# nquach/TEE_optical_flow

Hardware: AMD Instinct MI355X
Metric: frame-pairs/sec @512x512 DualTVL1 (higher is better)
Workload: dtype f32

## Files before the change

### tee_optical_flow_amd/csrc/teeflow.hip

```cpp
#include "teeflow_kernels.hip.h"
#include "teeflow_deepflow.hip.h"
#include "teeflow_sor_rt.hip.h"
#include "teeflow_analysis.hip.h"
#include "teeflow_wase.hip.h"
#include "teeflow_saliency.hip.h"
#include "teeflow_ccl.hip.h"
#include "teeflow_masks.hip.h"
#include "teeflow_otsu.hip.h"
#include "teeflow_centroid.hip.h"
#include "teeflow_area.hip.h"
#include "teeflow_polar.hip.h"
#include "teeflow_overlay.hip.h"
#include "teeflow_magoverlay.hip.h"
#include "teeflow_segmentor.hip.h"
#include "teeflow_inflate.hip.h"
#include "teeflow_deflate.hip.h"
#include "teeflow_ingest.hip.h"
#include "pil_resample_tables.h"
#include "../../include/teeflow.h"
#include "teeflow_engine.hip.h"
#include "teeflow_tvl1_host.hip.h"
#include "teeflow_deepflow_host.hip.h"
#include "teeflow_queue.hip.h"

// ... 102 lines not shown
        case TF_PARAM_EPSILON: *d = &p.epsilon; break;
        case TF_PARAM_INNER_ITERATIONS: *i = &p.inner_iterations; break;
        case TF_PARAM_OUTER_ITERATIONS: *i = &p.outer_iterations; break;
        case TF_PARAM_SCALE_STEP: *d = &p.scale_step; break;
        case TF_PARAM_GAMMA: *d = &p.gamma; break;
        case TF_PARAM_MEDIAN_FILTERING: *i = &p.median_filtering; break;
        case TF_PARAM_USE_INITIAL_FLOW: *i = &p.use_initial_flow; break;
        default: return false;
    }
    return true;
}

TF_API int tf_set_param(tf_handle* h, int key, double v)
{
    if (!h) return TF_ERR_INVALID_ARG;
    if (h->P.algo == TF_ALGO_DEEPFLOW) return fail(h, TF_ERR_UNSUPPORTED, "DeepFlow handles have creation-time parameters only (as cv2's object)");
    tf_params p = h->P;
    double* d; int* i;
    if (!param_field(p, key, &d, &i)) return fail(h, TF_ERR_INVALID_ARG, "unknown parameter key %d", key);
    if (d) *d = v; else *i = key == TF_PARAM_USE_INITIAL_FLOW ? v != 0.0 : (int)v;
    int rc = validate_params(h, p);
    if (rc) return rc;
    h->P = p;
    return TF_OK;
}

TF_API int tf_get_param(tf_handle* h, int key, double* v)
{
    if (!h || !v) return TF_ERR_INVALID_ARG;
    double* d; int* i;
    if (!param_field(h->P, key, &d, &i)) return fail(h, TF_ERR_INVALID_ARG, "unknown parameter key %d", key);
    *v = d ? *d : *i;
    return TF_OK;
}

TF_API int tf_set_stream(tf_handle* h, void* hip_stream, int use_external)
{
    if (!h) return TF_ERR_INVALID_ARG;
    HIPC(h, hipStreamSynchronize(h->stream));
    h->stream = use_external ? (hipStream_t)hip_stream : h->own_stream;
    return TF_OK;
}

TF_API int tf_set_tuning(tf_handle* h, const char* name, int value)
{
    if (!h || !name) return TF_ERR_INVALID_ARG;
    const std::string n(name);
    if (n == "iter_variant") {
        if (value < 0 || value > 2) return fail(h, TF_ERR_UNSUPPORTED, "iter_variant must be 0 (64x16 tiles), 1 (row strips) or 2 (row strips, two iterations per launch), got %d", value);
        h->iter_variant = value;
    }
    else if (n == "strip_blocks") h->strip_blocks = value > 0 ? value : 2048;
    else if (n == "min_rows_work") h->min_rows_work = value;
    else if (n == "lane_slots_pct") h->lane_slots_pct = value;
    else if (n == "sor_rt") h->sor_rt = value ? 1 : 0;
    else if (n == "sor_rt_shape") h->sor_rt_shape = value;
    else if (n == "sor_plain_div") h->sor_plain_div = value ? 1 : 0;
    else if (n == "max_strip_width") h->max_strip_width = value < 4 ? 4 : (value > 2048 ? 2048 : value);
    else if (n == "lanes") h->lanes = value < 1 ? 1 : (value > 8 ? 8 : value);
    else if (n == "queue_lanes") h->queue_lanes = value;
    else if (n == "queue_unit") h->queue_unit = value < 0 ? 0 : value;
    else if (n == "queue_test_fail_unit") h->queue_test_fail_unit = value;
    else if (n == "sor_fuse") h->sor_fuse = value;
    else if (n == "sor_coop") {
        h->sor_coop = value;
        if (value) { h->coop.rearm(); ++h->sor_coop_arm; }
    }
    else if (n == "sor_coop_s") h->sor_coop_s = value;
    else if (n == "sor_coop_small") h->sor_coop_small = value ? 1 : 0;
    else if (n == "sor_coop_min_util") h->sor_coop_min_util = value;
    else if (n == "coop_test_mute") h->coop_test_mute = value ? 1 : 0;
    else if (n == "coop_test_occ16") { h->coop_test_occ16 = value; h->coop.occ16 = -1; if (h->coop.flags) h->coop.query_occupancy(*h); }
    else if (n == "coop_test_occ8") { h->coop_test_occ8 = value; h->coop.occ16 = -1; if (h->coop.flags) h->coop.query_occupancy(*h); }
    else if (n == "coop_backoff") { h->coop.backoff = value < 0 ? 0 : value; }
    else if (n == "df_fuse_ds") h->df_fuse_ds = value < 0 ? 0 : (value > 2 ? 2 : value);
    else if (n == "warp_margin") h->warp_margin = value < 0 ? 0 : (value > 40 ? 40 : value);
    else if (n == "overlay_chunk_kib") h->overlay_chunk_kib = value < 0 ? 0 : (value > (512 << 10) ? (512 << 10) : value);
    else if (n == "area_chunk_kib") h->area_chunk_kib = value < 0 ? 0 : (value > (512 << 10) ? (512 << 10) : value);
    else return fail(h, TF_ERR_INVALID_ARG, "unknown tuning knob %s", name);
    return TF_OK;
}

#ifdef TF_COOP_TIMING
extern "C" __attribute__((visibility("default"))) int tf_dbg_coop_times(unsigned long long* out)
{
    return (int)hipMemcpyFromSymbol(out, HIP_SYMBOL(g_coop_t), sizeof(unsigned long long) * 4 * 64);
}
#endif
TF_API long long tf_dbg_counter(tf_handle* h, const char* name)
{
    if (!h || !name) return -1;
    const std::string n(name);
    long long v = -1;
    std::vector<CoopCounters> all{h->coop.counters()};
    if (h->pool) { std::lock_guard<std::mutex> lk(h->pool->m); all.insert(all.end(), h->pool->coop.begin(), h->pool->coop.end()); }
    if (n == "coop_launches") { v = 0; for (auto& c : all) v += c.launches; }
    else if (n == "coop_aborts") { v = 0; for (auto& c : all) v += c.aborts; }
    else if (n == "coop_disabled") { v = 0; for (auto& c : all) v |= (long long)c.disabled; }
    else if (n == "coop_rearms") { v = 0; for (auto& c : all) v += c.rearms; }
    else if (n == "coop_cooldown") { v = 0; for (auto& c : all) v = v > c.cooldown ? v : c.cooldown; }
    else if (n == "saliency_kernel_us") v = (long long)(h->pre_kernel_ms * 1000.0);
    else if (n == "wase_study_kernel_us") v = (long long)(h->wase_kernel_ms * 1000.0);
    else if (n == "inflate_kernel_us") v = (long long)(h->inflate_kernel_ms * 1000.0);
    else if (n == "unchunk_kernel_us") v = (long long)(h->unchunk_kernel_ms * 1000.0);
    else if (n == "deflate_match_us") v = (long long)(h->deflate_match_ms * 1000.0);
    else if (n == "deflate_emit_us") v = (long long)(h->deflate_emit_ms * 1000.0);
// ... 258 lines not shown
```

### tee_optical_flow_amd/csrc/teeflow_dbg.hip.h

```cpp
namespace {
template <class T> struct DevBuf { T* p = nullptr; ~DevBuf() { if (p) (void)hipFree(p); } };
using DBuf = DevBuf<float>;

int dbg_up(tf_handle* h, DBuf& d, const float* src, const Geom& g)
{
    HIPC(h, hipMalloc(&d.p, (size_t)g.plane * sizeof(float)));
    HIPC(h, hipMemsetAsync(d.p, 0, (size_t)g.plane * sizeof(float), h->stream));
    if (src) HIPC(h, hipMemcpy2DAsync(d.p, (size_t)g.pitch * 4, src, (size_t)g.w * 4, (size_t)g.w * 4, g.h, hipMemcpyHostToDevice, h->stream));
    return TF_OK;
}
int dbg_down(tf_handle* h, float* dst, const float* d, const Geom& g)
{
    HIPC(h, hipMemcpy2DAsync(dst, (size_t)g.w * 4, d, (size_t)g.pitch * 4, (size_t)g.w * 4, g.h, hipMemcpyDeviceToHost, h->stream));
    HIPC(h, hipStreamSynchronize(h->stream));
    return TF_OK;
}

int dbg_up2(tf_handle* h, DBuf& fr, const float* I0, const float* I1, const Geom& g)
{
    HIPC(h, hipMalloc(&fr.p, 2 * (size_t)g.plane * sizeof(float)));
    HIPC(h, hipMemsetAsync(fr.p, 0, 2 * (size_t)g.plane * sizeof(float), h->stream));
    HIPC(h, hipMemcpy2DAsync(fr.p, (size_t)g.pitch * 4, I0, (size_t)g.w * 4, (size_t)g.w * 4, g.h, hipMemcpyHostToDevice, h->stream));
    HIPC(h, hipMemcpy2DAsync(fr.p + g.plane, (size_t)g.pitch * 4, I1, (size_t)g.w * 4, (size_t)g.w * 4, g.h, hipMemcpyHostToDevice, h->stream));
    return TF_OK;
// ... 230 lines not shown
    const Geom g = make_geom(w, hgt);
    DBuf a0, a1, b0, b1;
    int rc;
    if ((rc = dbg_up(h, a0, src, g)) || (rc = dbg_up(h, a1, nullptr, g)) || (rc = dbg_up(h, b0, src, g)) || (rc = dbg_up(h, b1, nullptr, g))) return rc;
    DevBuf<PairCtl> ctl;
    HIPC(h, hipMalloc(&ctl.p, sizeof(PairCtl)));
    HIPC(h, hipMemsetAsync(ctl.p, 0, sizeof(PairCtl), h->stream));
    MedArgs ma = {};
    ma.sb.u1[0] = a0.p; ma.sb.u1[1] = a1.p; ma.sb.u2[0] = b0.p; ma.sb.u2[1] = b1.p;
    ma.ctl = ctl.p; ma.err = nullptr; ma.errstride = 0; ma.it = 0; ma.thr_q = 0; ma.utog = 0; ma.g = g;
    ma.total = 1; ma.step = iter_step(h, false, h->P.inner_iterations);
    const dim3 gm((g.w + 63) / 64, (g.h + 15) / 16, 2);
    if (ksize == 5) hipLaunchKernelGGL(k_median<5>, gm, dim3(256), 0, h->stream, ma);
    else hipLaunchKernelGGL(k_median<3>, gm, dim3(256), 0, h->stream, ma);
    hipError_t e = hipStreamSynchronize(h->stream);
    if (e != hipSuccess) return fail(h, TF_ERR_HIP, "k_median: %s", hipGetErrorString(e));
    return dbg_down(h, dst, a1.p, g);
}

TF_API int tf_dbg_iterate(tf_handle* h, const float* I1wx, const float* I1wy, const float* rho_c,
                          float* u1, float* u2, float* p11, float* p12, float* p21, float* p22,
                          int w, int hgt, int nsteps, int p_is_zero, unsigned long long* err_q)
{
    if (!h || !I1wx || !I1wy || !rho_c || !u1 || !u2 || !p11 || !p12 || !p21 || !p22 || w < 1 || hgt < 1 || nsteps < 0)
        return TF_ERR_INVALID_ARG;
    HIPC(h, hipSetDevice(h->dev));
    const Geom g = make_geom(w, hgt);
    DBuf cx, cy, cr, s[12];
    int rc;
    if ((rc = dbg_up(h, cx, I1wx, g)) || (rc = dbg_up(h, cy, I1wy, g)) || (rc = dbg_up(h, cr, rho_c, g))) return rc;
    float* hostp[6] = {u1, u2, p11, p12, p21, p22};
    for (int k = 0; k < 6; ++k) {
        if ((rc = dbg_up(h, s[2 * k], hostp[k], g)) || (rc = dbg_up(h, s[2 * k + 1], nullptr, g))) return rc;
    }
    DevBuf<PairCtl> ctl; DevBuf<u64> errs;
    HIPC(h, hipMalloc(&ctl.p, sizeof(PairCtl)));
    HIPC(h, hipMemsetAsync(ctl.p, 0, sizeof(PairCtl), h->stream));
    HIPC(h, hipMalloc(&errs.p, (size_t)(nsteps + 1) * sizeof(u64)));
    HIPC(h, hipMemsetAsync(errs.p, 0, (size_t)(nsteps + 1) * sizeof(u64), h->stream));
    Iter2Args A = {};
    IterArgs& ia = A.a;
    ia.wx = cx.p; ia.wy = cy.p; ia.rho = cr.p;
    for (int k = 0; k < 2; ++k) {
        ia.sb.u1[k] = s[0 + k].p; ia.sb.u2[k] = s[2 + k].p; ia.sb.p11[k] = s[4 + k].p;
        ia.sb.p12[k] = s[6 + k].p; ia.sb.p21[k] = s[8 + k].p; ia.sb.p22[k] = s[10 + k].p;
    }
    ia.ctl = ctl.p; ia.err = errs.p; ia.errstride = nsteps + 1; ia.thr_q = -1.0; ia.g = g; ia.host_slot = nullptr; ia.B = 1;
    ia.l_t = (float)(h->P.lambda * h->P.theta); ia.theta = (float)h->P.theta; ia.taut = (float)(h->P.tau / h->P.theta);
    const int step = iter_step(h, false, nsteps);
    A.total = nsteps;
    int launches = 0;
    for (int it = 0; it < nsteps; it += step, ++launches) {
        ia.it = it; ia.utog = ia.ptog = launches; ia.pzero = (p_is_zero && it == 0) ? 1 : 0;
        launch_iter(h, A, step, 1, h->stream);
    }
    hipError_t e = hipStreamSynchronize(h->stream);
    if (e == hipSuccess && err_q && nsteps > 0) {
        e = hipMemcpyAsync(err_q, errs.p, (size_t)nsteps * sizeof(u64), hipMemcpyDeviceToHost, h->stream);
        if (e == hipSuccess) e = hipStreamSynchronize(h->stream);
    }
    if (e != hipSuccess) return fail(h, TF_ERR_HIP, "k_iter: %s", hipGetErrorString(e));
    const int cur = launches & 1;
    for (int k = 0; k < 6; ++k)
        if ((rc = dbg_down(h, hostp[k], s[2 * k + cur].p, g))) return rc;
    return TF_OK;
}
```

### tee_optical_flow_amd/csrc/teeflow_engine.hip.h

```cpp
#include <rccl/rccl.h>
#include <algorithm>
#include <chrono>
#include <cmath>
#include <limits>
#include <cstdarg>
#include <cstdio>
#include <cstring>
#include <cstdlib>
#include <deque>
#include <string>
#include <atomic>
#include <condition_variable>
#include <mutex>
#include <thread>
#include <map>
#include <vector>

#define TF_API extern "C" __attribute__((visibility("default")))

namespace {
constexpr int MAXLEV = 64;
constexpr int DF_MAXLEV = 201;
constexpr int SLOT_RING = 1024;
constexpr int DEFAULT_LAG = 1;
constexpr int DEFAULT_MAX_BATCH = 128;

thread_local std::string g_create_error;

struct ProfEv { hipEvent_t a, b; int level = 0, warp = 0, it = 0; float ms = 0.f; double work = 0.0; };
}

namespace { struct Engine; }
struct LanePool;
struct QJob;
struct CoopCounters { long long launches = 0; int aborts = 0, rearms = 0, cooldown = 0; bool disabled = false; };
struct TfKnobs {
    int iter_variant = 2;
    int max_strip_width = 2048;
    int sor_rt = 1;
    int sor_plain_div = 0;
    int sor_rt_shape = 3;
    int df_fuse_ds = 2;
    int sor_coop = 1;
    int sor_coop_min_util = 85;
    int sor_coop_small = 1;
    int sor_coop_s = 5;
    int sor_fuse = 5;
    int warp_margin = 8;
    int min_rows_work = 8192;
    int strip_blocks = 2048;
    int lane_slots_pct = 67;
    int coop_test_occ16 = -1, coop_test_occ8 = -1;
    int coop_test_mute = 0;
    int profile = 0;
    int overlay_chunk_kib = 0;
    int area_chunk_kib = 0;
    unsigned sor_coop_arm = 0;
};

namespace {
struct Tvl1State {
    int H = 0, W = 0, cap = 0, nlev = 0;
    double scale_step = 0; int nscales = 0, variant = 0;
    Geom lv[MAXLEV];
    float* pyr[MAXLEV] = {};
    float* gxl[MAXLEV] = {}; float* gyl[MAXLEV] = {};
    float *cwx = nullptr, *cwy = nullptr, *crho = nullptr;
    StateBufs sb = {};
    PairCtl* ctl = nullptr;
    u64* errs = nullptr; int errstride = 0;
    int* iters_dev = nullptr; size_t iters_cap = 0;
    const void** chain_src = nullptr; size_t chain_src_cap = 0;
    volatile int* slots_host = nullptr; int* slots_dev = nullptr;
    unsigned launch_seq = 0;
    float* tab = nullptr;
    std::map<size_t, int> slots_cache;
    int ensure(Engine* e, int H, int W, int B);
    void release();
};

struct DfState {
    int nlev = 0, H = 0, W = 0, cap = 0;
    Geom lv[DF_MAXLEV];
    float* pyr_base = nullptr; size_t pyr_off[DF_MAXLEV] = {};
    float* tmp = nullptr;
    float* planes = nullptr;
    DfBufs bufs = {};
    int ensure(Engine* e, int H, int W, int B);
    void release();
};

struct Coop {
    int share = 0;
    bool disabled = false;
    int backoff = 0;
    int cooldown = 0;
    int rearms = 0;
    int occ16 = -1, occ8 = -1;
    int asked16 = -2, asked8 = -2;
    bool used = false;
    int aborts = 0;
    long long launches = 0;
    unsigned epoch = 0;
    unsigned* flags = nullptr;
    int flag_lines = 0;
    void tick();
    void query_occupancy(const TfKnobs& k);
    int ensure(Engine* e);
    int aborted(Engine* e, bool* aborted);
    void rearm() { disabled = false; backoff = cooldown = 0; }
    CoopCounters counters() const { return {launches, aborts, rearms, cooldown, disabled}; }
    void release();
};

struct Engine : TfKnobs {
    tf_params P;
    tf_deepflow_params DP = {};
    int dev = 0;
    int num_cus = 256;
    hipStream_t own_stream = nullptr, stream = nullptr;
    std::string err;
    hipStream_t copy_stream = nullptr;
    hipEvent_t cev[4] = {nullptr, nullptr, nullptr, nullptr};
    uint8_t* st_u8 = nullptr; size_t st_u8_bytes = 0;
    uint8_t* st_flow = nullptr; size_t st_flow_bytes = 0;
    uint8_t* st_init = nullptr; size_t st_init_bytes = 0;
    hipEvent_t ev[4] = {};
// ... 214 lines not shown
```

### tee_optical_flow_amd/csrc/teeflow_tvl1_host.hip.h

```cpp
namespace {
int validate_params(Engine* h, const tf_params& p)
{
    if (p.algo != TF_ALGO_TVL1) return fail(h, TF_ERR_UNSUPPORTED, "algo %d not implemented (only TF_ALGO_TVL1)", p.algo);
    if (p.nscales < 1 || p.nscales > MAXLEV) return fail(h, TF_ERR_INVALID_ARG, "nscales must be in [1,%d], got %d", MAXLEV, p.nscales);
    if (p.warps < 1) return fail(h, TF_ERR_INVALID_ARG, "warps must be >= 1, got %d", p.warps);
    if (p.inner_iterations < 1 || p.outer_iterations < 1)
        return fail(h, TF_ERR_INVALID_ARG, "inner/outer iterations must be >= 1, got %d/%d", p.inner_iterations, p.outer_iterations);
    if ((long long)p.inner_iterations * p.outer_iterations > 100000)
        return fail(h, TF_ERR_INVALID_ARG, "inner*outer iterations too large");
    if (p.median_filtering != 1 && p.median_filtering != 3 && p.median_filtering != 5)
        return fail(h, TF_ERR_UNSUPPORTED, "medianFiltering must be 1, 3 or 5 (cv::medianBlur on CV_32F), got %d", p.median_filtering);
    if (p.gamma != 0.0) return fail(h, TF_ERR_UNSUPPORTED, "gamma != 0 (illumination term u3) is not implemented");
    if (p.variant != TF_VARIANT_CPU && p.variant != TF_VARIANT_CUDA) return fail(h, TF_ERR_INVALID_ARG, "variant must be TF_VARIANT_CPU or TF_VARIANT_CUDA, got %d", p.variant);
    if (p.variant == TF_VARIANT_CUDA && (p.inner_iterations * p.outer_iterations) % 2 != 0)
        return fail(h, TF_ERR_UNSUPPORTED, "TF_VARIANT_CUDA needs an even iteration count (inner*outer), got %d", p.inner_iterations * p.outer_iterations);
    if (p.use_initial_flow && p.variant == TF_VARIANT_CUDA)
        return fail(h, TF_ERR_UNSUPPORTED, "useInitialFlow is not implemented for TF_VARIANT_CUDA (nothing checks that form bit for bit)");
    if (!(p.scale_step > 0.0 && p.scale_step < 1.0)) return fail(h, TF_ERR_INVALID_ARG, "scaleStep must be in (0,1), got %g", p.scale_step);
    if (p.scale_step == 0.5) return fail(h, TF_ERR_UNSUPPORTED, "scaleStep == 0.5 makes cv::resize take its INTER_AREA fast path for the pyramid, which is not implemented");
    if (!(p.theta > 0.0) || !(p.tau > 0.0) || !(p.lambda > 0.0) || !(p.epsilon >= 0.0))
        return fail(h, TF_ERR_INVALID_ARG, "tau, lambda, theta must be > 0 and epsilon >= 0");
    return TF_OK;
}

// ... 32 lines not shown
    HIPC(e, hipStreamSynchronize(e->stream));
    release(); release_staging(e);
    nlev = compute_levels(P, H_, W_, lv);
    const size_t ncap = (size_t)want_cap, fcap = 2 * ncap;
    for (int l = 0; l < nlev; ++l) HIPC(e, hipMalloc(&pyr[l], fcap * lv[l].plane * sizeof(float)));
    if (P.variant == TF_VARIANT_CUDA)
        for (int l = 0; l < nlev; ++l) {
            HIPC(e, hipMalloc(&gxl[l], fcap * lv[l].plane * sizeof(float)));
            HIPC(e, hipMalloc(&gyl[l], fcap * lv[l].plane * sizeof(float)));
        }
    variant = P.variant;
    const size_t pl = (size_t)lv[0].plane * ncap * sizeof(float);
    HIPC(e, hipMalloc(&cwx, pl)); HIPC(e, hipMalloc(&cwy, pl)); HIPC(e, hipMalloc(&crho, pl));
    for (int k = 0; k < 2; ++k) {
        HIPC(e, hipMalloc(&sb.u1[k], pl)); HIPC(e, hipMalloc(&sb.u2[k], pl));
        HIPC(e, hipMalloc(&sb.p11[k], pl)); HIPC(e, hipMalloc(&sb.p12[k], pl));
        HIPC(e, hipMalloc(&sb.p21[k], pl)); HIPC(e, hipMalloc(&sb.p22[k], pl));
    }
    HIPC(e, hipMalloc(&ctl, ncap * sizeof(PairCtl)));
    errstride = total;
    HIPC(e, hipMalloc(&errs, ncap * (size_t)errstride * sizeof(u64)));
    iters_cap = ncap * (size_t)nlev * (size_t)P.warps * 2;
    HIPC(e, hipMalloc(&iters_dev, iters_cap * sizeof(int)));
    H = H_; W = W_; cap = want_cap;
    scale_step = P.scale_step; nscales = P.nscales;
    return TF_OK;
}

inline dim3 grid64x4(const Geom& g, int z) { return dim3((g.w + 63) / 64, (g.h + 3) / 4, z); }

bool rows_ok(const Engine* h, const Geom& g, int B)
{
    return h->iter_variant >= 1 && g.w <= h->max_strip_width && (long long)g.h * B >= h->min_rows_work;
}

int iter_step(const Engine* h, bool cuda_variant, int inner)
{
    return (cuda_variant || (h->iter_variant >= 2 && inner % 2 == 0)) ? 2 : 1;
}

void strip_shape(const Engine* h, const Geom& g, int B, int* R, int* QX, int* RY, int* threads)
{
    const int qx = (g.w + 3) / 4;
    int ry = 256 / qx;
    if (ry < 1) ry = 1;
    *QX = qx; *RY = ry;
    *threads = qx * ry <= 256 ? 256 : (qx * ry + 63) / 64 * 64;
    long long n = (long long)g.h * B / ((long long)h->strip_blocks * ry);
    if (n < 2) n = 2;
    if (n > 16) n = 16;
    *R = ry * (int)n;
}

void launch_iter(Engine* h, const Iter2Args& A, int step, int B, hipStream_t s)
{
    const Geom& g = A.a.g;
    if (!rows_ok(h, g, B)) {
        if (step == 2) hipLaunchKernelGGL(k_iter2_tile, dim3((g.w + T2_OW - 1) / T2_OW, (g.h + T2_OH - 1) / T2_OH, B), dim3(256), 0, s, A);
        else hipLaunchKernelGGL(k_iter, dim3((g.w + IT_OW - 1) / IT_OW, (g.h + IT_OH - 1) / IT_OH, B), dim3(256), 0, s, A.a);
        return;
    }
    int R, QX, RY, threads;
    strip_shape(h, g, B, &R, &QX, &RY, &threads);
    const int LW = QX * 4 + 4;
    if (step == 1) {
        const size_t shmem1 = (size_t)(32 + 8 * RY * LW + 2 * RY * QX) * sizeof(float);
        hipLaunchKernelGGL(k_iter_rows, dim3((g.h + R - 1) / R, 1, B), dim3(threads), shmem1, s, A.a, R, QX, RY);
        return;
    }
    const size_t shmem = (size_t)(32 + 8 * RY * LW + 2 * (RY + 1) * LW + 2 * RY * QX) * sizeof(float);
    if (B <= 1024) {
        auto f = h->tv.slots_cache.find(shmem * 1024 + (size_t)threads / 64);
        if (f == h->tv.slots_cache.end()) {
            int per_cu = 0;
            (void)hipOccupancyMaxActiveBlocksPerMultiprocessor(&per_cu, k_iter2_rows, threads, shmem);
            if (per_cu < 1) per_cu = 1;
            f = h->tv.slots_cache.emplace(shmem * 1024 + (size_t)threads / 64, per_cu * h->num_cus).first;
        }
        int slots = f->second;
        if (h->slots_pct > 0 && h->slots_pct < 100) slots = slots * h->slots_pct / 100;
        int items = 1;
        for (int n = 1; n <= B; ++n) {
            int r, sn;
            strip_rule(n, g.h, RY, slots, &r, &sn);
            if (n * sn > items) items = n * sn;
        }
        hipLaunchKernelGGL(k_iter2_rows, dim3(items, 1, 1), dim3(threads), shmem, s, A, 0, QX, RY, slots);
        return;
    }
    hipLaunchKernelGGL(k_iter2_rows, dim3((g.h + R - 1) / R, 1, B), dim3(threads), shmem, s, A, R, QX, RY, 0);
}

inline int warp_margin_class(int m) { return m <= 0 ? 0 : (m <= 4 ? 4 : (m <= 8 ? 8 : 16)); }
void launch_warp(Engine* h, const WarpArgs& wa, int B, hipStream_t s, const float* gx = nullptr, const float* gy = nullptr)
{
    const Geom& g = wa.g;
    if (h->P.variant == TF_VARIANT_CUDA) {
        WarpCudaArgs ca; ca.w = wa; ca.gx = gx; ca.gy = gy;
        hipLaunchKernelGGL(k_warp_cuda, dim3((g.w + 63) / 64, (g.h + 3) / 4, B), dim3(256), 0, s, ca);
        return;
    }
    const int M = warp_margin_class(h->warp_margin);
    const dim3 grid((g.w + WL_TW - 1) / WL_TW, (g.h + WL_TH - 1) / WL_TH, B);
    const size_t shm = (size_t)(128 + (WL_TW + 2 * (M + 4)) * (WL_TH + 2 * M + 7)) * sizeof(float);
    switch (M) {
        case 4: hipLaunchKernelGGL(k_warp_lds<4>, grid, dim3(256), shm, s, wa); break;
        case 8: hipLaunchKernelGGL(k_warp_lds<8>, grid, dim3(256), shm, s, wa); break;
        case 16: hipLaunchKernelGGL(k_warp_lds<16>, grid, dim3(256), shm, s, wa); break;
        default: hipLaunchKernelGGL(k_warp, dim3((g.w + 63) / 64, (g.h + 3) / 4, B), dim3(256), 0, s, wa); break;
    }
}

int read_reports(Engine* h, hipStream_t s, unsigned q, unsigned* checked, bool* stop)
{
    while (*checked <= q) {
        int v = h->tv.slots_host[*checked % SLOT_RING];
        if (v < 0) {
            if (q - *checked < (unsigned)DEFAULT_LAG) break;
            const double t0 = now_ms();
            while ((v = h->tv.slots_host[*checked % SLOT_RING]) < 0) {
                if (now_ms() - t0 > 20000.0) return fail(h, TF_ERR_HIP, "tvl1_iter launch %u never reported (GPU hang?)", *checked);
                if (hipStreamQuery(s) == hipSuccess && h->tv.slots_host[*checked % SLOT_RING] < 0)
                    return fail(h, TF_ERR_HIP, "stream drained but launch %u did not report", *checked);
            }
        }
        ++*checked;
        if (v == 0) { *stop = true; break; }
    }
    return TF_OK;
}

int run_stage(Engine* h, int l, int wi, int B, int off0, int off1, int* iters_dev)
{
    const tf_params& P = h->P;
    const Geom g = h->tv.lv[l];
    const int inner = P.inner_iterations, total = P.inner_iterations * P.outer_iterations;
    const float thr_f = (float)(P.epsilon * P.epsilon * (double)(g.w * g.h));
    const double thr_q = (double)thr_f * 1073741824.0;
    const double thr_d = P.epsilon * P.epsilon * (double)(g.w * g.h);
    hipStream_t s = h->stream;

    WarpArgs wa;
    wa.pyr = h->tv.pyr[l]; wa.off0 = off0; wa.off1 = off1; wa.sb = h->tv.sb; wa.ctl = h->tv.ctl; wa.tab = h->tv.tab;
    wa.wx = h->tv.cwx; wa.wy = h->tv.cwy; wa.rho = h->tv.crho; wa.g = g;
    int rc = profiled(h, s, -4, 0, 0, [&] { launch_warp(h, wa, B, s, h->tv.gxl[l], h->tv.gyl[l]); });
    if (rc) return rc;
    HIPC(h, hipMemsetAsync(h->tv.errs, 0, (size_t)B * h->tv.errstride * sizeof(u64), s));

    Iter2Args A;
    IterArgs& ia = A.a;
    ia.wx = h->tv.cwx; ia.wy = h->tv.cwy; ia.rho = h->tv.crho; ia.sb = h->tv.sb; ia.ctl = h->tv.ctl; ia.err = h->tv.errs;
    ia.errstride = h->tv.errstride; ia.thr_q = thr_q; ia.g = g;
    ia.l_t = (float)(P.lambda * P.theta); ia.theta = (float)P.theta; ia.taut = (float)(P.tau / P.theta);
    ia.variant = P.variant; ia.thr_d = thr_d;
    const bool cuda_variant = P.variant == TF_VARIANT_CUDA;
    const bool median = P.median_filtering > 1 && !cuda_variant;
    MedArgs ma;
    ma.sb = h->tv.sb; ma.ctl = h->tv.ctl; ma.err = h->tv.errs; ma.errstride = h->tv.errstride; ma.thr_q = thr_q; ma.g = g;

    const dim3 gm((g.w + 63) / 64, (g.h + 15) / 16, 2 * B);
    ia.B = B;
    const int step = iter_step(h, cuda_variant, inner);
    ma.total = A.total = total; ma.step = step;
    A.utog_prev = A.ptog_prev = A.pzero_prev = 0;
    int utog = 0, ptog = 0;
    bool stop = false;
    unsigned checked = h->tv.launch_seq;
    for (int it = 0; it < total + step - 1 && !stop; it += step) {
        if (it < total && it % inner == 0 && median) {
            ma.it = it; ma.utog = utog;
            rc = profiled(h, s, -5, 0, 0, [&] {
                if (P.median_filtering == 5) hipLaunchKernelGGL(k_median<5>, gm, dim3(256), 0, s, ma);
                else hipLaunchKernelGGL(k_median<3>, gm, dim3(256), 0, s, ma);
            });
            if (rc) return rc;
            ++utog;
        }
        const unsigned q = h->tv.launch_seq++;
        h->tv.slots_host[q % SLOT_RING] = -1;
        ia.host_slot = h->tv.slots_dev + q % SLOT_RING;
        ia.it = it; ia.utog = utog; ia.ptog = ptog; ia.pzero = (wi == 0 && it == 0) ? 1 : 0;
        rc = profiled(h, s, l, wi, it, [&] { launch_iter(h, A, step, B, s); });
        if (rc) return rc;
        ++h->tally.iter_launches;
        A.utog_prev = utog; A.ptog_prev = ptog; A.pzero_prev = ia.pzero;
        ++utog; ++ptog;
        rc = read_reports(h, s, q, &checked, &stop);
        if (rc) return rc;
    }
    hipLaunchKernelGGL(k_stage_end, dim3((B + 255) / 256), dim3(256), 0, s, h->tv.errs, h->tv.errstride, h->tv.ctl, iters_dev, B,
                       total, inner, median ? 1 : 0, thr_q, l, wi, h->tv.nlev, P.warps, P.variant, thr_d, step);
    return TF_OK;
}

void pyramids_below_level0(Engine* h, int F)
{
    const tf_params& P = h->P;
    hipStream_t s = h->stream;
    for (int l = 1; l < h->tv.nlev; ++l) {
        const double sc = 1.0 / P.scale_step;
        hipLaunchKernelGGL(k_pyr_down, grid64x4(h->tv.lv[l], F), dim3(256), 0, s, h->tv.pyr[l - 1], h->tv.lv[l - 1], h->tv.pyr[l], h->tv.lv[l], sc, sc,
                           P.variant == TF_VARIANT_CUDA ? 1 : 0);
    }
    if (P.variant == TF_VARIANT_CUDA)
        for (int l = 0; l < h->tv.nlev; ++l)
            hipLaunchKernelGGL(k_grad, grid64x4(h->tv.lv[l], F), dim3(256), 0, s, h->tv.pyr[l], h->tv.gxl[l], h->tv.gyl[l], h->tv.lv[l]);
}

void build_pyramids(Engine* h, const uint8_t* dframes, bool f32, int F)
{
    hipStream_t s = h->stream;
    const Geom g0 = h->tv.lv[0];
    if (f32) hipLaunchKernelGGL(k_f32_to_level0, dim3((g0.w + 255) / 256, g0.h, F), dim3(256), 0, s, (const float*)dframes, h->tv.pyr[0], g0, 1);
    else hipLaunchKernelGGL(k_u8_to_f32, dim3((g0.w + 255) / 256, g0.h, F), dim3(256), 0, s, dframes, h->tv.pyr[0], g0);
    pyramids_below_level0(h, F);
}

enum Seed { SEED_ZERO, SEED_FLOWS, SEED_STATE };

int solve_pairs(Engine* h, int B, int off0, int off1, Seed seed, const float* dinit, int* iters_dev, float scale, void* dflow, bool out_f16)
{
    const tf_params& P = h->P;
    hipStream_t s = h->stream;
    const Geom g0 = h->tv.lv[0];
    const int L = h->tv.nlev - 1;
    const auto seed_step = [&](int l) {
        if (l > 0) hipLaunchKernelGGL(k_init_down, grid64x4(h->tv.lv[l], B), dim3(256), 0, s, h->tv.sb, (L - l + 1) & 1, h->tv.lv[l - 1], h->tv.lv[l],
                                      1.0 / P.scale_step, (float)P.scale_step);
        else if (seed == SEED_FLOWS) hipLaunchKernelGGL(k_init_split, grid64x4(g0, B), dim3(256), 0, s, dinit, h->tv.sb, L & 1, g0);
    };
    if (seed == SEED_STATE)
        hipLaunchKernelGGL(k_chain_seed, dim3((g0.pitch + 63) / 64, (g0.h + 3) / 4, B), dim3(256), 0, s, h->tv.sb, h->tv.ctl, L & 1, g0, L == 0 ? 1 : 0);
    hipLaunchKernelGGL(k_ctl_set, dim3((B + 255) / 256), dim3(256), 0, s, h->tv.ctl, B, 0);
    if (seed != SEED_ZERO) for (int l = 0; l < L; ++l) seed_step(l);
    if (!(seed == SEED_STATE && L == 0)) {
        HIPC(h, hipMemset2DAsync(h->tv.sb.u1[0], (size_t)h->tv.lv[L].splane * sizeof(float), 0, (size_t)h->tv.lv[L].plane * sizeof(float), B, s));
        HIPC(h, hipMemset2DAsync(h->tv.sb.u2[0], (size_t)h->tv.lv[L].splane * sizeof(float), 0, (size_t)h->tv.lv[L].plane * sizeof(float), B, s));
    }
    if (seed != SEED_ZERO) seed_step(L);
    for (int l = L; l >= 0; --l) {
        for (int wi = 0; wi < P.warps; ++wi) {
            int rc = run_stage(h, l, wi, B, off0, off1, iters_dev);
            if (rc) return rc;
        }
        if (l == 0) break;
        const Geom gs = h->tv.lv[l], gd = h->tv.lv[l - 1];
        const double sx = 1.0 / ((double)gd.w / gs.w), sy = 1.0 / ((double)gd.h / gs.h);
        hipLaunchKernelGGL(k_flow_up, grid64x4(gd, B), dim3(256), 0, s, h->tv.sb, h->tv.ctl, gs, gd, sx, sy, (float)(1 / P.scale_step),
                           P.variant == TF_VARIANT_CUDA ? 1 : 0);
        hipLaunchKernelGGL(k_ctl_set, dim3((B + 255) / 256), dim3(256), 0, s, h->tv.ctl, B, 1);
    }
    if (out_f16) hipLaunchKernelGGL(k_output<uint16_t>, out_grid<uint16_t>(g0, B), dim3(256), 0, s, h->tv.sb, h->tv.ctl, g0, scale, (uint16_t*)dflow);
    else hipLaunchKernelGGL(k_output<float>, out_grid<float>(g0, B), dim3(256), 0, s, h->tv.sb, h->tv.ctl, g0, scale, (float*)dflow);
    HIPC(h, hipGetLastError());
    return TF_OK;
}

int solve_resident(Engine* h, const uint8_t* dframes, bool f32, int F, int B, int off0, int off1, float scale, void* dflow, bool out_f16,
                   const float* dinit = nullptr)
{
    build_pyramids(h, dframes, f32, F);
    return solve_pairs(h, B, off0, off1, dinit ? SEED_FLOWS : SEED_ZERO, dinit, h->tv.iters_dev, scale, dflow, out_f16);
}

int solve_chain_resident(Engine* h, const uint8_t* dframes, bool f32, int B, float scale, void* dflow, bool out_f16, bool carry)
{
    build_pyramids(h, dframes, f32, B + 1);
    const size_t per_pair = (size_t)h->tv.nlev * h->P.warps * 2;
    const size_t flb = (size_t)h->tv.H * h->tv.W * 2 * (out_f16 ? sizeof(uint16_t) : sizeof(float));
    for (int k = 0; k < B; ++k) {
        const int rc = solve_pairs(h, 1, k, k + 1, k > 0 || carry ? SEED_STATE : SEED_ZERO, nullptr, h->tv.iters_dev + (size_t)k * per_pair, scale,
                                   (uint8_t*)dflow + (size_t)k * flb, out_f16);
        if (rc) return rc;
        ++h->tally.chain_steps;
    }
    return TF_OK;
}

int solve_chains_resident(Engine* h, const void* const* dsrc, bool f32, int S, int T, const int* Bk, float scale, void* dflow, bool out_f16, bool carry)
{
    const Geom g0 = h->tv.lv[0];
    const int F = (T + 1) * S;
    hipLaunchKernelGGL(k_chain_gather, dim3((g0.w + 255) / 256, g0.h, F), dim3(256), 0, h->stream, dsrc, f32 ? 1 : 0, h->tv.pyr[0], g0);
    pyramids_below_level0(h, F);
    const size_t per_pair = (size_t)h->tv.nlev * h->P.warps * 2;
    const size_t flb = (size_t)h->tv.H * h->tv.W * 2 * (out_f16 ? sizeof(uint16_t) : sizeof(float));
    for (int k = 0; k < T; ++k) {
        const int rc = solve_pairs(h, Bk[k], k * S, (k + 1) * S, k > 0 || carry ? SEED_STATE : SEED_ZERO, nullptr,
                                   h->tv.iters_dev + (size_t)k * S * per_pair, scale, (uint8_t*)dflow + (size_t)k * S * flb, out_f16);
        if (rc) return rc;
        h->tally.chain_steps += Bk[k];
    }
    return TF_OK;
}

void account_bytes(const Engine* h, const int* it , bool seeded, double* iter_bytes, double* total_bytes,
                   unsigned long long* n_in, unsigned long long* n_out)
{
    const int warps = h->P.warps;
    double ib = 0, tb = 0;
    for (int l = 0; l < h->tv.nlev; ++l) {
        const double px = (double)h->tv.lv[l].w * h->tv.lv[l].h;
        for (int w = 0; w < warps; ++w) {
// ... 16 lines not shown
```

### tee_optical_flow_amd/csrc/teeflow_tvl1_iter.hip.h

```cpp
#pragma once

__device__ __forceinline__ bool pair_active(const u64* errb, int it, double thr_q)
{
    if (it == 0) return true;
    return (double)errb[it - 1] > thr_q;
}

#define IT_TW 64
#define IT_TH 16
#define IT_OW 60
#define IT_OH 15

struct IterArgs {
    const float *wx, *wy, *rho;
    StateBufs sb;
    const PairCtl* ctl;
    u64* err; int errstride; int it; double thr_q;
    int utog, ptog, pzero;
    Geom g;
    float l_t, theta, taut;
    int* host_slot;
    int B;
    int variant;
    double thr_d;
// ... 748 lines not shown
                const unsigned mnl = opaque_u(lastrow ? 0u : ~0u);
                float dv1[4], dv2[4], r11[4], r12[4], r21[4], r22[4], u1x[4], u1y[4], u2x[4], u2y[4];
                UNPACK4(dv1, dn1) UNPACK4(dv2, dn2)
                {
                    const float4 o1 = ld4(U2a + (bq * RY + ty) * LW + x), o2 = ld4(U2b + (bq * RY + ty) * LW + x);
                    UNPACK4(s2_u1, o1) UNPACK4(s2_u2, o2)
                }
#pragma unroll
                for (int i = 0; i < 4; ++i) {
                    const float e1 = i < 3 ? s2_u1[i + 1] : rr1, e2 = i < 3 ? s2_u2[i + 1] : rr2;
                    u1x[i] = mask_f(e1 - s2_u1[i], inw[i + 1]);
                    u2x[i] = mask_f(e2 - s2_u2[i], inw[i + 1]);
                    u1y[i] = mask_f(dv1[i] - s2_u1[i], mnl);
                    u2y[i] = mask_f(dv2[i] - s2_u2[i], mnl);
                }
                tv_p_quad_pk(a.taut, u1x, u1y, u2x, u2y, s2_11, s2_12, s2_21, s2_22, r11, r12, r21, r22);
                const size_t prow = (size_t)yc * pitch + x;
                st4(ou1 + prow, PACK4(s2_u1)); st4(ou2 + prow, PACK4(s2_u2));
                st4(o11 + prow, PACK4(r11)); st4(o12 + prow, PACK4(r12));
                st4(o21 + prow, PACK4(r21)); st4(o22 + prow, PACK4(r22));
            }
        }
        else __syncthreads();
        s2_valid = v2u;
#pragma unroll
        for (int i = 0; i < 4; ++i) {
            s2_11[i] = p1_11[i]; s2_12[i] = p1_12[i]; s2_21[i] = p1_21[i]; s2_22[i] = p1_22[i];
            s1_wx[i] = wxv[i]; s1_wy[i] = wyv[i]; s1_r[i] = rv[i];
            s1_11[i] = c11[i]; s1_12[i] = c12[i]; s1_21[i] = c21[i]; s1_22[i] = c22[i];
        }
        s1_valid = v1;
        ring += RY; ring = ring >= RB ? ring - RB : ring;
        if ((s & 255) == 255) { qA += (u64)accA; qB += (u64)accB; accA = accB = 0.0; }
    }
    if (!replay) {
        qA += (u64)accA; qB += (u64)accB;
#pragma unroll
        for (int off = 32; off > 0; off >>= 1) { qA += __shfl_down(qA, off, 64); qB += __shfl_down(qB, off, 64); }
        __syncthreads();
        if ((tid & 63) == 0) { sred[tid >> 6] = qA; sred[8 + (tid >> 6)] = qB; }
        __syncthreads();
        if (tid == 0) {
            u64 ta = 0, tb = 0;
            for (int w = 0; w < (int)(blockDim.x >> 6); ++w) { ta += sred[w]; tb += sred[8 + w]; }
            atomicAdd(&errb[k.it], ta);
            atomicAdd(&errb[k.it + 1], tb);
        }
    }
}

#define T2_OW 52
#define T2_OH 13

__global__ __launch_bounds__(256) void k_iter2_tile(Iter2Args A)
{
    constexpr int LW = 68;
    __shared__ __attribute__((aligned(16))) float sA[16][LW], sB[16][LW];
    __shared__ __attribute__((aligned(16))) float s12[16][LW], s22[16][LW];
    __shared__ float s11w[16][16], s21w[16][16];
    __shared__ u64 sred[8];
    const IterArgs& a = A.a;
    publish_active_count2(A);
    const int b = blockIdx.z;
    u64* errb = a.err + (size_t)b * a.errstride;
    const int mode = pair_mode(errb, a.it, A.total, a.thr_q, a.variant, a.thr_d);
    if (mode == M_EXIT) return;
    const bool replay = mode == M_REPLAY;
    const PairCtl c = a.ctl[b];
    const int utog = replay ? A.utog_prev : a.utog, ptog = replay ? A.ptog_prev : a.ptog;
    const bool pzero = (replay ? A.pzero_prev : a.pzero) != 0;
    const int uc = (c.ubase ^ utog) & 1, pc = (c.pbase ^ ptog) & 1;
    const int tx = threadIdx.x & 15, ty = threadIdx.x >> 4;
    const int W = a.g.w, H = a.g.h, pitch = a.g.pitch;
    const int x = (int)blockIdx.x * T2_OW - 4 + tx * 4, y = (int)blockIdx.y * T2_OH - 1 + ty;
    const bool inr = x >= 0 && x < W && y >= 0 && y < H;
    const bool outq = inr && tx >= 1 && tx <= 13 && ty >= 1 && ty <= 13;
    const size_t po = (size_t)b * a.g.splane;
    const size_t row = po + (size_t)(inr ? y : 0) * pitch + (inr ? x : 0);

    unsigned inw[5];
#pragma unroll
    for (int j = 0; j < 5; ++j) inw[j] = opaque_u(x + j < W ? ~0u : 0u);
    const unsigned mnl = opaque_u(y >= H - 1 ? 0u : ~0u);
    const unsigned mout = opaque_u(outq ? ~0u : 0u);
    const unsigned keep[4] = {inw[0] & mout, inw[1] & mout, inw[2] & mout, inw[3] & mout};

    float u0_1[4], u0_2[4], wx[4], wy[4], rc[4], p0_11[4], p0_12[4], p0_21[4], p0_22[4];
    float u1_1[4], u1_2[4];
    double accA = 0.0, accB = 0.0;
    if (inr) {
        const float4 u1q = ld4(a.sb.u1[uc] + row), u2q = ld4(a.sb.u2[uc] + row);
        const float4 wxq = ld4(a.wx + row), wyq = ld4(a.wy + row), rq = ld4(a.rho + row);
        float4 a11 = make_float4(0, 0, 0, 0), a12 = a11, a21 = a11, a22 = a11, up12 = a11, up22 = a11;
        float l11 = 0.f, l21 = 0.f;
        if (!pzero) {
            a11 = ld4(a.sb.p11[pc] + row); a12 = ld4(a.sb.p12[pc] + row);
            a21 = ld4(a.sb.p21[pc] + row); a22 = ld4(a.sb.p22[pc] + row);
            if (y > 0) { up12 = ld4(a.sb.p12[pc] + row - pitch); up22 = ld4(a.sb.p22[pc] + row - pitch); }
            if (x > 0) { l11 = a.sb.p11[pc][row - 1]; l21 = a.sb.p21[pc][row - 1]; }
        }
        QuadU qu;
        UNPACK4(qu.u1k, u1q) UNPACK4(qu.u2k, u2q) UNPACK4(qu.wx, wxq) UNPACK4(qu.wy, wyq) UNPACK4(qu.r, rq)
        UNPACK4(qu.p11, a11) UNPACK4(qu.p12, a12) UNPACK4(qu.p21, a21) UNPACK4(qu.p22, a22)
        UNPACK4(qu.p12u, up12) UNPACK4(qu.p22u, up22)
        qu.l11 = l11; qu.l21 = l21;
        UNPACK4(u0_1, u1q) UNPACK4(u0_2, u2q) UNPACK4(wx, wxq) UNPACK4(wy, wyq) UNPACK4(rc, rq)
        UNPACK4(p0_11, a11) UNPACK4(p0_12, a12) UNPACK4(p0_21, a21) UNPACK4(p0_22, a22)
        tv_u_quad_pk(a.l_t, a.theta, qu, y == 0, x == 0, u1_1, u1_2);
        if (!replay) accA += tv_err_quad_pk(u1_1, u0_1, u1_2, u0_2, keep);
        st4(&sA[ty][tx * 4], PACK4(u1_1));
        st4(&sB[ty][tx * 4], PACK4(u1_2));
    }
    __syncthreads();
    float p1_11[4], p1_12[4], p1_21[4], p1_22[4];
    const bool vP1 = inr && tx <= 14 && ty <= 14;
    if (vP1) {
        const float4 dn1 = ld4(&sA[ty + 1][tx * 4]), dn2 = ld4(&sB[ty + 1][tx * 4]);
        const float rr1 = sA[ty][tx * 4 + 4], rr2 = sB[ty][tx * 4 + 4];
        float dv1[4], dv2[4], u1x[4], u1y[4], u2x[4], u2y[4];
        UNPACK4(dv1, dn1) UNPACK4(dv2, dn2)
#pragma unroll
        for (int i = 0; i < 4; ++i) {
            const float e1 = i < 3 ? u1_1[i + 1] : rr1, e2 = i < 3 ? u1_2[i + 1] : rr2;
            u1x[i] = mask_f(e1 - u1_1[i], inw[i + 1]); u2x[i] = mask_f(e2 - u1_2[i], inw[i + 1]);
            u1y[i] = mask_f(dv1[i] - u1_1[i], mnl); u2y[i] = mask_f(dv2[i] - u1_2[i], mnl);
        }
        tv_p_quad_pk(a.taut, u1x, u1y, u2x, u2y, p0_11, p0_12, p0_21, p0_22, p1_11, p1_12, p1_21, p1_22);
// ... 7 lines not shown
            st4(&s12[ty][tx * 4], PACK4(p1_12));
            st4(&s22[ty][tx * 4], PACK4(p1_22));
            s11w[ty][tx] = p1_11[3];
            s21w[ty][tx] = p1_21[3];
        }
    }
    if (replay) return;
    __syncthreads();
    float u2_1[4], u2_2[4];
    const bool vU2 = vP1 && tx >= 1 && ty >= 1;
    if (vU2) {
        const float4 up12 = ld4(&s12[ty - 1][tx * 4]), up22 = ld4(&s22[ty - 1][tx * 4]);
        QuadU qu;
#pragma unroll
        for (int i = 0; i < 4; ++i) {
            qu.u1k[i] = u1_1[i]; qu.u2k[i] = u1_2[i]; qu.wx[i] = wx[i]; qu.wy[i] = wy[i]; qu.r[i] = rc[i];
            qu.p11[i] = p1_11[i]; qu.p12[i] = p1_12[i]; qu.p21[i] = p1_21[i]; qu.p22[i] = p1_22[i];
        }
        UNPACK4(qu.p12u, up12) UNPACK4(qu.p22u, up22)
        qu.l11 = s11w[ty][tx - 1]; qu.l21 = s21w[ty][tx - 1];
        tv_u_quad_pk(a.l_t, a.theta, qu, y == 0, x == 0, u2_1, u2_2);
        accB += tv_err_quad_pk(u2_1, u1_1, u2_2, u1_2, keep);
        st4(&sA[ty][tx * 4], PACK4(u2_1));
        st4(&sB[ty][tx * 4], PACK4(u2_2));
    }
    __syncthreads();
    if (outq) {
        const float4 dn1 = ld4(&sA[ty + 1][tx * 4]), dn2 = ld4(&sB[ty + 1][tx * 4]);
        const float rr1 = sA[ty][tx * 4 + 4], rr2 = sB[ty][tx * 4 + 4];
        float dv1[4], dv2[4], u1x[4], u1y[4], u2x[4], u2y[4], o11[4], o12[4], o21[4], o22[4];
        UNPACK4(dv1, dn1) UNPACK4(dv2, dn2)
#pragma unroll
        for (int i = 0; i < 4; ++i) {
            const float e1 = i < 3 ? u2_1[i + 1] : rr1, e2 = i < 3 ? u2_2[i + 1] : rr2;
            u1x[i] = mask_f(e1 - u2_1[i], inw[i + 1]); u2x[i] = mask_f(e2 - u2_2[i], inw[i + 1]);
            u1y[i] = mask_f(dv1[i] - u2_1[i], mnl); u2y[i] = mask_f(dv2[i] - u2_2[i], mnl);
        }
        tv_p_quad_pk(a.taut, u1x, u1y, u2x, u2y, p1_11, p1_12, p1_21, p1_22, o11, o12, o21, o22);
        st4(a.sb.u1[uc ^ 1] + row, PACK4(u2_1)); st4(a.sb.u2[uc ^ 1] + row, PACK4(u2_2));
        st4(a.sb.p11[pc ^ 1] + row, PACK4(o11)); st4(a.sb.p12[pc ^ 1] + row, PACK4(o12));
        st4(a.sb.p21[pc ^ 1] + row, PACK4(o21)); st4(a.sb.p22[pc ^ 1] + row, PACK4(o22));
    }
    u64 qA = (u64)accA, qB = (u64)accB;
#pragma unroll
    for (int off = 32; off > 0; off >>= 1) { qA += __shfl_down(qA, off, 64); qB += __shfl_down(qB, off, 64); }
    if ((threadIdx.x & 63) == 0) { sred[threadIdx.x >> 6] = qA; sred[4 + (threadIdx.x >> 6)] = qB; }
    __syncthreads();
    if (threadIdx.x == 0) {
        atomicAdd(&errb[a.it], sred[0] + sred[1] + sred[2] + sred[3]);
        atomicAdd(&errb[a.it + 1], sred[4] + sred[5] + sred[6] + sred[7]);
    }
}

__global__ void k_stage_end(const u64* __restrict__ err, int errstride, PairCtl* ctl, int* iters, int B,
                            int total, int inner, int median_on, double thr_q, int level, int warp, int nlev, int warps,
                            int variant, double thr_d, int step)
{
    const int b = blockIdx.x * blockDim.x + threadIdx.x;
    if (b >= B) return;
    const u64* e = err + (size_t)b * errstride;
    int n_it = total;
    if (variant) (void)pair_mode_cuda(e, total, total, thr_d, &n_it);
    else
        for (int j = 0; j < total; ++j)
            if (!((double)e[j] > thr_q)) { n_it = j + 1; break; }
    const int n_out = variant ? 0 : (n_it > 0 ? (n_it - 1) / inner + 1 : 0);
    const int launches = step == 2 ? (n_it + 1) / 2 : n_it;
    PairCtl c = ctl[b];
    c.ubase = (c.ubase + launches + (median_on ? n_out : 0)) & 1;
    c.pbase = (c.pbase + launches) & 1;
    ctl[b] = c;
    int* o = iters + (((size_t)b * nlev + level) * warps + warp) * 2;
    o[0] = n_it; o[1] = n_out;
}

__global__ void k_ctl_set(PairCtl* ctl, int B, int mode)
{
    const int b = blockIdx.x * blockDim.x + threadIdx.x;
    if (b >= B) return;
    if (mode == 0) { ctl[b].ubase = 0; ctl[b].pbase = 0; }
    else { ctl[b].ubase ^= 1; ctl[b].pbase = 0; }
}
```

Before: 2825.

## Compact TV-L1 iteration grid to active pairs and fold error-buffer clears into kernels

Adds a compacted tile kernel that launches tiles only for the number of still-active pairs (read back from host reports) and maps each block to the k-th active pair through ballot masks. It is gated by a new thin_rows_work knob that defaults to 0, so the compacted path is off by default. Separately, the per-warp-stage hipMemsetAsync of the error buffer is replaced by zeroing inside k_stage_end and k_ctl_set, and k_stage_end now scans the convergence errors with a 64-lane ballot instead of a serial loop. This removes one memset launch per stage, at the cost of one 64-thread block per pair for these small kernels.

After: 2837 (median of 6 runs). Within noise of the previous version (+0.4%).

```diff
diff --git a/tee_optical_flow_amd/csrc/teeflow.hip b/tee_optical_flow_amd/csrc/teeflow.hip
--- a/tee_optical_flow_amd/csrc/teeflow.hip
+++ b/tee_optical_flow_amd/csrc/teeflow.hip
@@ -178,6 +178,7 @@
     }
     else if (n == "strip_blocks") h->strip_blocks = value > 0 ? value : 2048;
     else if (n == "min_rows_work") h->min_rows_work = value;
+    else if (n == "thin_rows_work") h->thin_rows_work = value < 0 ? 0 : value;
     else if (n == "lane_slots_pct") h->lane_slots_pct = value;
     else if (n == "sor_rt") h->sor_rt = value ? 1 : 0;
     else if (n == "sor_rt_shape") h->sor_rt_shape = value;
diff --git a/tee_optical_flow_amd/csrc/teeflow_dbg.hip.h b/tee_optical_flow_amd/csrc/teeflow_dbg.hip.h
--- a/tee_optical_flow_amd/csrc/teeflow_dbg.hip.h
+++ b/tee_optical_flow_amd/csrc/teeflow_dbg.hip.h
@@ -306,7 +306,7 @@
     int launches = 0;
     for (int it = 0; it < nsteps; it += step, ++launches) {
         ia.it = it; ia.utog = ia.ptog = launches; ia.pzero = (p_is_zero && it == 0) ? 1 : 0;
-        launch_iter(h, A, step, 1, h->stream);
+        launch_iter(h, A, step, 1, INT_MAX, h->stream);
     }
     hipError_t e = hipStreamSynchronize(h->stream);
     if (e == hipSuccess && err_q && nsteps > 0) {
diff --git a/tee_optical_flow_amd/csrc/teeflow_engine.hip.h b/tee_optical_flow_amd/csrc/teeflow_engine.hip.h
--- a/tee_optical_flow_amd/csrc/teeflow_engine.hip.h
+++ b/tee_optical_flow_amd/csrc/teeflow_engine.hip.h
@@ -48,6 +48,7 @@
     int sor_fuse = 5;
     int warp_margin = 8;
     int min_rows_work = 8192;
+    int thin_rows_work = 0;
     int strip_blocks = 2048;
     int lane_slots_pct = 67;
     int coop_test_occ16 = -1, coop_test_occ8 = -1;
@@ -73,6 +74,7 @@
     const void** chain_src = nullptr; size_t chain_src_cap = 0;
     volatile int* slots_host = nullptr; int* slots_dev = nullptr;
     unsigned launch_seq = 0;
+    int n_max = 0;
     float* tab = nullptr;
     std::map<size_t, int> slots_cache;
     int ensure(Engine* e, int H, int W, int B);
diff --git a/tee_optical_flow_amd/csrc/teeflow_tvl1_host.hip.h b/tee_optical_flow_amd/csrc/teeflow_tvl1_host.hip.h
--- a/tee_optical_flow_amd/csrc/teeflow_tvl1_host.hip.h
+++ b/tee_optical_flow_amd/csrc/teeflow_tvl1_host.hip.h
@@ -108,9 +108,14 @@
     *R = ry * (int)n;
 }
 
-void launch_iter(Engine* h, const Iter2Args& A, int step, int B, hipStream_t s)
+void launch_iter(Engine* h, const Iter2Args& A, int step, int B, int n_max, hipStream_t s)
 {
     const Geom& g = A.a.g;
+    if (step == 2 && B <= 1024 && (long long)n_max * g.h < h->thin_rows_work) {
+        const int tiles_x = (g.w + T2_OW - 1) / T2_OW, tiles = tiles_x * ((g.h + T2_OH - 1) / T2_OH);
+        hipLaunchKernelGGL(k_iter2_tile_act, dim3(tiles * (n_max > 1 ? n_max : 1)), dim3(256), 0, s, A, tiles_x, tiles);
+        return;
+    }
     if (!rows_ok(h, g, B)) {
         if (step == 2) hipLaunchKernelGGL(k_iter2_tile, dim3((g.w + T2_OW - 1) / T2_OW, (g.h + T2_OH - 1) / T2_OH, B), dim3(256), 0, s, A);
         else hipLaunchKernelGGL(k_iter, dim3((g.w + IT_OW - 1) / IT_OW, (g.h + IT_OH - 1) / IT_OH, B), dim3(256), 0, s, A.a);
@@ -181,6 +186,7 @@
             }
         }
         ++*checked;
+        h->tv.n_max = v;
         if (v == 0) { *stop = true; break; }
     }
     return TF_OK;
@@ -201,7 +207,6 @@
     wa.wx = h->tv.cwx; wa.wy = h->tv.cwy; wa.rho = h->tv.crho; wa.g = g;
     int rc = profiled(h, s, -4, 0, 0, [&] { launch_warp(h, wa, B, s, h->tv.gxl[l], h->tv.gyl[l]); });
     if (rc) return rc;
-    HIPC(h, hipMemsetAsync(h->tv.errs, 0, (size_t)B * h->tv.errstride * sizeof(u64), s));
 
     Iter2Args A;
     IterArgs& ia = A.a;
@@ -221,6 +226,7 @@
     A.utog_prev = A.ptog_prev = A.pzero_prev = 0;
     int utog = 0, ptog = 0;
     bool stop = false;
+    h->tv.n_max = B;
     unsigned checked = h->tv.launch_seq;
     for (int it = 0; it < total + step - 1 && !stop; it += step) {
         if (it < total && it % inner == 0 && median) {
@@ -236,7 +242,7 @@
         h->tv.slots_host[q % SLOT_RING] = -1;
         ia.host_slot = h->tv.slots_dev + q % SLOT_RING;
         ia.it = it; ia.utog = utog; ia.ptog = ptog; ia.pzero = (wi == 0 && it == 0) ? 1 : 0;
-        rc = profiled(h, s, l, wi, it, [&] { launch_iter(h, A, step, B, s); });
+        rc = profiled(h, s, l, wi, it, [&] { launch_iter(h, A, step, B, h->tv.n_max, s); });
         if (rc) return rc;
         ++h->tally.iter_launches;
         A.utog_prev = utog; A.ptog_prev = ptog; A.pzero_prev = ia.pzero;
@@ -244,7 +250,7 @@
         rc = read_reports(h, s, q, &checked, &stop);
         if (rc) return rc;
     }
-    hipLaunchKernelGGL(k_stage_end, dim3((B + 255) / 256), dim3(256), 0, s, h->tv.errs, h->tv.errstride, h->tv.ctl, iters_dev, B,
+    hipLaunchKernelGGL(k_stage_end, dim3(B), dim3(64), 0, s, h->tv.errs, h->tv.errstride, h->tv.ctl, iters_dev, B,
                        total, inner, median ? 1 : 0, thr_q, l, wi, h->tv.nlev, P.warps, P.variant, thr_d, step);
     return TF_OK;
 }
@@ -287,7 +293,7 @@
     };
     if (seed == SEED_STATE)
         hipLaunchKernelGGL(k_chain_seed, dim3((g0.pitch + 63) / 64, (g0.h + 3) / 4, B), dim3(256), 0, s, h->tv.sb, h->tv.ctl, L & 1, g0, L == 0 ? 1 : 0);
-    hipLaunchKernelGGL(k_ctl_set, dim3((B + 255) / 256), dim3(256), 0, s, h->tv.ctl, B, 0);
+    hipLaunchKernelGGL(k_ctl_set, dim3(B), dim3(64), 0, s, h->tv.ctl, B, 0, h->tv.errs, h->tv.errstride);
     if (seed != SEED_ZERO) for (int l = 0; l < L; ++l) seed_step(l);
     if (!(seed == SEED_STATE && L == 0)) {
         HIPC(h, hipMemset2DAsync(h->tv.sb.u1[0], (size_t)h->tv.lv[L].splane * sizeof(float), 0, (size_t)h->tv.lv[L].plane * sizeof(float), B, s));
@@ -304,7 +310,7 @@
         const double sx = 1.0 / ((double)gd.w / gs.w), sy = 1.0 / ((double)gd.h / gs.h);
         hipLaunchKernelGGL(k_flow_up, grid64x4(gd, B), dim3(256), 0, s, h->tv.sb, h->tv.ctl, gs, gd, sx, sy, (float)(1 / P.scale_step),
                            P.variant == TF_VARIANT_CUDA ? 1 : 0);
-        hipLaunchKernelGGL(k_ctl_set, dim3((B + 255) / 256), dim3(256), 0, s, h->tv.ctl, B, 1);
+        hipLaunchKernelGGL(k_ctl_set, dim3(B), dim3(64), 0, s, h->tv.ctl, B, 1, h->tv.errs, h->tv.errstride);
     }
     if (out_f16) hipLaunchKernelGGL(k_output<uint16_t>, out_grid<uint16_t>(g0, B), dim3(256), 0, s, h->tv.sb, h->tv.ctl, g0, scale, (uint16_t*)dflow);
     else hipLaunchKernelGGL(k_output<float>, out_grid<float>(g0, B), dim3(256), 0, s, h->tv.sb, h->tv.ctl, g0, scale, (float*)dflow);
diff --git a/tee_optical_flow_amd/csrc/teeflow_tvl1_iter.hip.h b/tee_optical_flow_amd/csrc/teeflow_tvl1_iter.hip.h
--- a/tee_optical_flow_amd/csrc/teeflow_tvl1_iter.hip.h
+++ b/tee_optical_flow_amd/csrc/teeflow_tvl1_iter.hip.h
@@ -824,7 +824,7 @@
 #define T2_OW 52
 #define T2_OH 13
 
-__global__ __launch_bounds__(256) void k_iter2_tile(Iter2Args A)
+__device__ __forceinline__ void iter2_tile_body(const Iter2Args& A, const int b, const int bx, const int by)
 {
     constexpr int LW = 68;
     __shared__ __attribute__((aligned(16))) float sA[16][LW], sB[16][LW];
@@ -832,8 +832,6 @@
     __shared__ float s11w[16][16], s21w[16][16];
     __shared__ u64 sred[8];
     const IterArgs& a = A.a;
-    publish_active_count2(A);
-    const int b = blockIdx.z;
     u64* errb = a.err + (size_t)b * a.errstride;
     const int mode = pair_mode(errb, a.it, A.total, a.thr_q, a.variant, a.thr_d);
     if (mode == M_EXIT) return;
@@ -844,7 +842,7 @@
     const int uc = (c.ubase ^ utog) & 1, pc = (c.pbase ^ ptog) & 1;
     const int tx = threadIdx.x & 15, ty = threadIdx.x >> 4;
     const int W = a.g.w, H = a.g.h, pitch = a.g.pitch;
-    const int x = (int)blockIdx.x * T2_OW - 4 + tx * 4, y = (int)blockIdx.y * T2_OH - 1 + ty;
+    const int x = bx * T2_OW - 4 + tx * 4, y = by * T2_OH - 1 + ty;
     const bool inr = x >= 0 && x < W && y >= 0 && y < H;
     const bool outq = inr && tx >= 1 && tx <= 13 && ty >= 1 && ty <= 13;
     const size_t po = (size_t)b * a.g.splane;
@@ -958,32 +956,84 @@
     }
 }
 
-__global__ void k_stage_end(const u64* __restrict__ err, int errstride, PairCtl* ctl, int* iters, int B,
-                            int total, int inner, int median_on, double thr_q, int level, int warp, int nlev, int warps,
-                            int variant, double thr_d, int step)
-{
-    const int b = blockIdx.x * blockDim.x + threadIdx.x;
+__global__ __launch_bounds__(256) void k_iter2_tile(Iter2Args A)
+{
+    publish_active_count2(A);
+    iter2_tile_body(A, (int)blockIdx.z, (int)blockIdx.x, (int)blockIdx.y);
+}
+
+__device__ __forceinline__ int active_pair_masks(const Iter2Args& A, u64* masks)
+{
+    const IterArgs& a = A.a;
+    const int nchunk = (a.B + 63) >> 6, nw = (int)(blockDim.x >> 6), wv = (int)(threadIdx.x >> 6), ln = (int)(threadIdx.x & 63);
+    for (int c = wv; c < nchunk; c += nw) {
+        const int pb = c * 64 + ln;
+        const bool on = pb < a.B && pair_mode(a.err + (size_t)pb * a.errstride, a.it, A.total, a.thr_q, a.variant, a.thr_d) != M_EXIT;
+        const u64 m = __ballot(on);
+        if (ln == 0) masks[c] = m;
+    }
+    __syncthreads();
+    int nact = 0;
+    for (int c = 0; c < nchunk; ++c) nact += __popcll(masks[c]);
+    return nact;
+}
+
+__device__ __forceinline__ int kth_active_pair(const u64* masks, int k)
+{
+    int c = 0;
+    u64 m = masks[0];
+    while (k >= __popcll(m)) { k -= __popcll(m); m = masks[++c]; }
+    for (; k > 0; --k) m &= m - 1;
+    return c * 64 + (__ffsll((long long)m) - 1);
+}
+
+__global__ __launch_bounds__(256) void k_iter2_tile_act(Iter2Args A, int tiles_x, int tiles_per_pair)
+{
+    __shared__ u64 smask[16];
+    publish_active_count2(A);
+    const int nact = active_pair_masks(A, smask);
+    const int k = (int)blockIdx.x / tiles_per_pair;
+    if (k >= nact) return;
+    const int t = (int)blockIdx.x - k * tiles_per_pair;
+    const int ty = t / tiles_x;
+    iter2_tile_body(A, kth_active_pair(smask, k), t - ty * tiles_x, ty);
+}
+
+__global__ __launch_bounds__(64) void k_stage_end(u64* err, int errstride, PairCtl* ctl, int* iters, int B,
+                                                  int total, int inner, int median_on, double thr_q, int level, int warp, int nlev, int warps,
+                                                  int variant, double thr_d, int step)
+{
+    const int b = blockIdx.x, ln = threadIdx.x;
     if (b >= B) return;
-    const u64* e = err + (size_t)b * errstride;
+    u64* e = err + (size_t)b * errstride;
     int n_it = total;
     if (variant) (void)pair_mode_cuda(e, total, total, thr_d, &n_it);
     else
-        for (int j = 0; j < total; ++j)
-            if (!((double)e[j] > thr_q)) { n_it = j + 1; break; }
-    const int n_out = variant ? 0 : (n_it > 0 ? (n_it - 1) / inner + 1 : 0);
-    const int launches = step == 2 ? (n_it + 1) / 2 : n_it;
-    PairCtl c = ctl[b];
-    c.ubase = (c.ubase + launches + (median_on ? n_out : 0)) & 1;
-    c.pbase = (c.pbase + launches) & 1;
-    ctl[b] = c;
-    int* o = iters + (((size_t)b * nlev + level) * warps + warp) * 2;
-    o[0] = n_it; o[1] = n_out;
-}
-
-__global__ void k_ctl_set(PairCtl* ctl, int B, int mode)
-{
-    const int b = blockIdx.x * blockDim.x + threadIdx.x;
+        for (int j0 = 0; j0 < total; j0 += 64) {
+            const int j = j0 + ln;
+            const u64 m = __ballot(j < total && !((double)e[j] > thr_q));
+            if (m) { n_it = j0 + __ffsll((long long)m); break; }
+        }
+    if (ln == 0) {
+        const int n_out = variant ? 0 : (n_it > 0 ? (n_it - 1) / inner + 1 : 0);
+        const int launches = step == 2 ? (n_it + 1) / 2 : n_it;
+        PairCtl c = ctl[b];
+        c.ubase = (c.ubase + launches + (median_on ? n_out : 0)) & 1;
+        c.pbase = (c.pbase + launches) & 1;
+        ctl[b] = c;
+        int* o = iters + (((size_t)b * nlev + level) * warps + warp) * 2;
+        o[0] = n_it; o[1] = n_out;
+    }
+    for (int j = ln; j < errstride; j += 64) e[j] = 0;
+}
+
+__global__ __launch_bounds__(64) void k_ctl_set(PairCtl* ctl, int B, int mode, u64* err, int errstride)
+{
+    const int b = blockIdx.x, ln = threadIdx.x;
     if (b >= B) return;
-    if (mode == 0) { ctl[b].ubase = 0; ctl[b].pbase = 0; }
-    else { ctl[b].ubase ^= 1; ctl[b].pbase = 0; }
-}
+    if (mode == 0) {
+        if (ln == 0) { ctl[b].ubase = 0; ctl[b].pbase = 0; }
+        for (int j = ln; j < errstride; j += 64) err[(size_t)b * errstride + j] = 0;
+    }
+    else if (ln == 0) { ctl[b].ubase ^= 1; ctl[b].pbase = 0; }
+}
```
